# logv/sybil

Hardware: AMD Instinct MI355X
Metric: rows scanned/sec (1B-row x 32-int-col synthetic table, 3 ANDed int-range filters, group-by 2 cols, count/sum/avg/stddev of 2 cols) (higher is better)
Workload: dtype int64

## Files before the change

### sybil_amd/csrc/engine.cpp

```cpp
#include "engine.h"
#include "hll.h"
#include "re2lite.h"

#include <math.h>
#include <stdarg.h>
#include <stdio.h>
#include <stdlib.h>
#include <string.h>

#include <algorithm>
#include <mutex>
#include <unordered_map>
#include <string>
#include <vector>
#include <regex>

namespace sybl {

extern "C" char **environ;
const char *env(const char *name) {
    static std::unordered_map<std::string, std::string> snap;
    static bool live = false;
    static std::once_flag once;
    std::call_once(once, [] {
// ... 60 lines not shown
    if (e != hipSuccess) return e;
    return hipStreamCreateWithPriority(out, hipStreamNonBlocking, toward < 0 ? greatest : least);
}

static void free_query(Query *q) {
    if (!q) return;
    if (!q->table_gone) {
        query_finish_lazy_results(q);
        if (q->t) {
            auto &v = q->t->queries;
            v.erase(std::remove(v.begin(), v.end(), q), v.end());
        }
    }
    q->eff_weight.reset();
    q->fword.reset();
    if (q->d_plan) hipFree(q->d_plan);
    if (q->d_preplan) hipFree(q->d_preplan);
    if (q->d_prebits) hipFree(q->d_prebits);
    if (q->d_segs) hipFree(q->d_segs);
    if (q->d_wg_seg_begin) hipFree(q->d_wg_seg_begin);
    if (q->d_pieces) hipFree(q->d_pieces);
    if (q->d_piece_queue) hipFree(q->d_piece_queue);
    if (q->d_wg_cell_base) hipFree(q->d_wg_cell_base);
    if (q->d_recs) hipFree(q->d_recs);
    if (q->d_h32) hipFree(q->d_h32);
    if (q->d_cursor) hipFree(q->d_cursor);
    for (void *p : q->d_idmasks) hipFree(p);
    if (q->own_partials) {
        if (q->d_sum) hipFree(q->d_sum);
        if (q->d_max) hipFree(q->d_max);
// ... 645 lines not shown
```

### sybil_amd/csrc/engine.h

```cpp
#pragma once
#include <hip/hip_runtime.h>
#include <stdint.h>

#include <map>
#include <atomic>
#include <functional>
#include <memory>
#include <mutex>
#include <string>
#include <unordered_map>
#include <string.h>
#include <stdio.h>
#include <stdlib.h>
#include <algorithm>
#include <chrono>
#include <thread>
#include <vector>

#include "../../include/sybilgpu.h"
#include "plan.h"
#include "scan_fast.h"
#include "scan_packed.h"
#include "fword.h"

// ... 118 lines not shown
    std::vector<int64_t> h_set_off;
    std::vector<int32_t> h_set_vals;
    bool set_dirty = false;
    void *d_stage = nullptr;
    int64_t stage_cap = 0;
};

struct LoadedBlock {
    std::string name;
    int64_t mtime_ns = 0, size = 0;
    int64_t index = -1;
};

struct FilterWord {
    std::vector<int> cols;
    int n = 0;
    int32_t bits[kFwordMaxFields] = {}, shift[kFwordMaxFields] = {};
    int elem[kFwordMaxFields] = {};
    int64_t vbase[kFwordMaxFields] = {};
    void *d_data = nullptr;
    int64_t cap_rows = 0;
    int64_t rows = 0, version = -1, blocks = 0;
    uint64_t planned = 0;
    ~FilterWord() {
        if (d_data) (void)hipFree(d_data);
    }
};

struct Query;
struct Table {
// ... 12 lines not shown
    int64_t scratch_words = 0;
    int64_t version = 0;
    int64_t broken_blocks = 0;
    sybl_load_stats load_stats{};
    sybl_digest_stats digest_stats{};
    sybl_select_stats select_stats{};
    sybl_concat_stats concat_stats{};
    sybl_lookup_stats lookup_stats{};
    sybl_compute_stats compute_stats{};
    std::string src_dir;
    int src_rank = 0, src_nranks = 1;
    std::vector<LoadedBlock> loaded;
    std::vector<Query *> queries;
    std::vector<std::shared_ptr<FilterWord>> fwords;
    uint64_t fword_clock = 0;
    Column *find(const char *name) const;
};

int table_ensure_stats(Table *t);
int table_reserve(Table *t, Column *c, int64_t phys_rows);
int valid_reserve(Table *t, Column *c, int64_t phys_rows);
int64_t table_drop_dead_tail(Table *t, int64_t keep_blocks);
int table_upload_blocks(Table *t);
int table_reclaim_dead_rows(Table *t, bool force);
void column_free(Column *c);
int32_t dict_intern(Column *c, const std::string &s);
int column_upload_set(Table *t, Column *c);
int column_build_gdict(Table *t, Column *c);
int column_build_rank(Table *t, Column *c);
Column *column_build_narrow(Table *t, Column *c);
void column_drop_narrow(Column *c);
std::shared_ptr<FilterWord> table_build_fword(Table *t, const int *cols, int n);
int column_install_gdict(Table *t, Column *c);
int column_repack(Table *t, Column *c, int width, int64_t vbase);

struct BlockWriter {
    Table *t = nullptr;
    int64_t start = 0, nrows = 0, new_phys = 0;
    struct Staged {
        Column *c = nullptr;
        bool have_stats = false;
        int64_t mn = 0, mx = 0, pop = 0;
    };
    std::vector<Staged> staged;
    std::vector<Staged> direct;
    bool serial = false;
};
// ... 140 lines not shown
    ScanPlan dplan;
    ScanPlan *d_dplan = nullptr;
    uint8_t *d_hll = nullptr;
    uint64_t *d_hll_idhash = nullptr;
    char *d_hll_chars = nullptr;
    int64_t *d_hll_stroff = nullptr;
    int64_t hll_bytes = 0;
    bool distinct_pending = false;
    bool time_mode = false;
    int64_t time_bucket = 0;
    std::string order_by;
    bool order_asc = false;
    int limit = 0;
    std::shared_ptr<Column> eff_weight;
    std::shared_ptr<FilterWord> fword;
    int printed_level = 0;
    bool printed_only = false;
    bool top_only = false;
    bool top_merge = false;
    std::vector<GroupInfo> groups;
    std::vector<AggInfo> aggs;
    ScanPlan plan;
    ScanPlan *d_plan = nullptr;
    bool plan_dirty = true;
    int n_wg = 0;
    bool use_lds = false;
    size_t lds_bytes = 0;
    int64_t group_cells = 0;
    std::vector<Segment> segs;
    std::vector<int32_t> wg_seg_begin;
// ... 171 lines not shown
```

### sybil_amd/csrc/fword.h

```cpp
#pragma once
#ifdef __HIPCC__
#include <hip/hip_runtime.h>
#endif
#include <stdint.h>

#ifndef SYBL_HD
#ifdef __HIPCC__
#define SYBL_HD __host__ __device__ __forceinline__
#else
#define SYBL_HD inline
#endif
#endif

namespace sybl {

constexpr int kFwordMaxFields = 4;
constexpr int kFwordMinFields = 2;
constexpr int kFwordBits = 32;

SYBL_HD int fword_bits(uint32_t max_off) {
    int b = 1;
    while (b < 32 && (max_off >> b) != 0) b++;
    return b;
}
// ... 6 lines not shown
        total += bits[i];
    }
    return total;
}

SYBL_HD uint32_t fword_mask(int bits) { return (1u << bits) - 1u; }

SYBL_HD uint32_t fword_pack(const uint32_t *offsets, int n, const int32_t *shifts) {
    uint32_t w = 0;
    for (int i = 0; i < n; i++) w |= offsets[i] << shifts[i];
    return w;
}

SYBL_HD uint32_t fword_field(uint32_t word, int shift, int bits) { return (word >> shift) & fword_mask(bits); }

struct FwordPack {
    const void *col[kFwordMaxFields];
    int32_t wid[kFwordMaxFields];
    int32_t shift[kFwordMaxFields], bits[kFwordMaxFields];
    int32_t n;
};

}
```

### sybil_amd/csrc/planner.cpp

```cpp
#include <math.h>
#include <stdlib.h>
#include <string.h>

#include <algorithm>

#include "engine.h"
#include "hll.h"
#include "re2lite.h"

namespace sybl {

static inline int64_t round_up(int64_t x, int64_t m) { return (x + m - 1) / m * m; }


struct HostFilterFold {
    bool has_range = false;
    int64_t lo = INT64_MIN, hi = INT64_MAX;
    std::vector<int64_t> neq;
    bool has_mask = false;
    std::vector<uint8_t> mask;
    std::vector<std::pair<int32_t, int32_t>> setp;
};

static void setup_buckets(int64_t info_min, int64_t info_max, int64_t hist_bucket, int64_t *bucket_size,
// ... 1539 lines not shown
            if (cols[c] < 0) return;
            const Column *col = t->cols[(size_t)cols[c]].get();
            if (FP.fmask[c] || FP.nneq[c] || FP.npneq[c] || FP.fvalid[c] || FP.fwid[c] != col->elem || FP.fbase[c] != col->vbase) return;
        }
        std::shared_ptr<FilterWord> w = table_build_fword(t, cols, q->fast_nf);
        if (!w) return;
        for (int c = 0; c < q->fast_nf; c++) {
            const int i = (int)(std::find(w->cols.begin(), w->cols.end(), cols[c]) - w->cols.begin());
            FP.fshift[c] = w->shift[i];
            FP.fbits[c] = w->bits[i];
        }
        FP.fword = (const uint32_t *)w->d_data;
        q->fword = std::move(w);
    }

    void plan_narrow() {
        if (!(q->fast && q->fast_packed && !q->fast_packed_n && !q->hash_mode && !q->part_hist)) return;
        FastPlan &FP = q->fplan;
        plan_fword();
        for (int a = 0; a < q->fast_na; a++) {
            Column *c = t->cols[(size_t)q->aggs[(size_t)a].col].get();
            if (FP.awid[a] != 4 || (const void *)FP.acol[a] != c->d_data || FP.abase[a] != c->vbase) continue;
            if (Column *n = column_build_narrow(t, c)) {
                FP.acol[a] = (const int64_t *)n->d_data;
                FP.awid[a] = n->elem;
            }
        }
        if (env("SYBL_PLAN_TRACE")) {
            int bytes = q->time_mode ? FP.twid : 0;
            for (int c = 0; c < q->fast_nf; c++) bytes += FP.fword ? 0 : FP.fwid[c];
            for (int c = 0; c < q->fast_ng; c++) bytes += FP.gwid[c];
            std::string line = "narrow:";
            if (FP.fword) {
                bytes += 4;
                line += " f=word(";
                for (int c = 0; c < q->fast_nf; c++) line += (c ? "," : "") + std::to_string(FP.fbits[c]);
                line += ")";
            }
            for (int a = 0; a < q->fast_na; a++) {
                bytes += FP.awid[a];
                line += " a" + std::to_string(a) + "=" + std::to_string(FP.awid[a]);
            }
            fprintf(stderr, "%s bytes_per_row=%d\n", line.c_str(), bytes);
        }
    }

    int plan_pushdown() {
        q->pushdown = false;
        q->pd_static = q->printed_level == 2 && !env("SYBL_NO_PUSHDOWN") && !env("SYBL_NO_PUSHDOWN_RANKS") && q->limit > 0 && q->order_by == "$COUNT" &&
                       !q->order_asc && d->n_groups == 1 && d->n_filters == 0 && d->op == SYBL_AGG_HIST && d->n_aggs >= 1 && d->n_aggs <= 2 &&
                       d->n_distincts == 0 && ctx->comm && ctx->comm_nranks > 1;
        q->pd_agreed = -1;
        if (q->printed_level != 2 || env("SYBL_NO_PUSHDOWN")) return SYBL_OK;
        if (!q->part_hist || !q->part_packed || !q->part_more.empty() || q->part_nf != 0 || q->part_ng != 1) return SYBL_OK;
// ... 379 lines not shown
```

### sybil_amd/csrc/scan_fast.h

```cpp
#pragma once
#include <hip/hip_runtime.h>
#include <stdint.h>

#include "plan.h"
#include "pieces.h"
#include "outlog.h"
#include "wg_header.h"

namespace sybl {

constexpr int kFastMaxF = 4, kFastMaxG = 4, kFastMaxA = 4;
constexpr int kFastTemplatedG = 2, kFastTemplatedA = 2;

enum FastMode : int {
    kFastAvg = 0,
    kFastAvgMax = 1,
    kFastMoments = 2,
    kFastHist = 3,
    kFastModes = 4,
};

struct FastPlan {
    const int64_t *fcol[kFastMaxF];
    const int64_t *gcol[kFastMaxG];
// ... 44 lines not shown
    int32_t nul;
    int32_t lds_sum_fields;
    const int32_t *wg_cell_base;
    const uint32_t *xvalid;
    int64_t *out_log;
    int64_t out_cap;
    int64_t *sum_out, *max_out, *ws_sum, *ws_max;
    const Segment *segs;
    const int32_t *wg_seg_begin;
    unsigned long long *wg_clock;
    int32_t dyn, n_pieces, piece_cap;
    const Piece *pieces;
    uint32_t *piece_queue;
    const uint32_t *fword;
    int32_t fshift[kFastMaxF], fbits[kFastMaxF];
};

hipError_t launch_scan_fast(const FastPlan &P, int nf, int ng, int na, int mode, bool time, bool gen, int n_wg,
                            size_t lds_bytes, hipStream_t st);

inline bool fast_plan_has_narrow(const FastPlan &P, bool aggs) {
    bool any = P.twid == 3 || P.wwid == 3;
    for (int c = 0; c < kFastMaxF; c++) any = any || P.fwid[c] == 3;
    for (int c = 0; c < kFastMaxG; c++) any = any || P.gwid[c] == 3;
    for (int c = 0; aggs && c < kFastMaxA; c++) any = any || P.awid[c] == 3;
    return any;
}

constexpr uint32_t kLeanMoments = 1u, kLeanProved = 2u;
constexpr int lean_sum_fields(int na) { return na + (na + 1) / 2 + na; }
constexpr int lean_bits(unsigned __int128 x) {
    int b = 0;
    while (x) b++, x >>= 1;
    return b;
}
constexpr int lean_moments_fit(int na, const uint64_t *umax, const uint64_t *bmax, unsigned __int128 slot_rows) {
    const unsigned __int128 one = 1;
// ... 1103 lines not shown
```

### sybil_amd/csrc/scan_packed.h

```cpp
#pragma once
#include "narrow3.h"
#include "fword.h"
#include "scan_fast.h"

namespace sybl {

constexpr int kPackedRows = 4;
constexpr int kPackedTileRows = kWgThreads * kPackedRows;

hipError_t launch_scan_packed(const FastPlan &P, int nf, int ng, int na, int mode, bool time, int n_wg, size_t lds_bytes,
                              hipStream_t st);
hipError_t launch_emit_packed(const EmitPlan &E, int nf, int ng, int na, int n_wg, hipStream_t st);
hipError_t launch_count_packed_nf0(const EmitPlan &E, int ng, int n_wg, hipStream_t st);
hipError_t launch_count_packed_nf1(const EmitPlan &E, int ng, int n_wg, hipStream_t st);
hipError_t launch_count_packed_nf2(const EmitPlan &E, int ng, int n_wg, hipStream_t st);
hipError_t launch_count_packed_nf3(const EmitPlan &E, int ng, int n_wg, hipStream_t st);
hipError_t launch_count_packed_nf4(const EmitPlan &E, int ng, int n_wg, hipStream_t st);
hipError_t launch_emit_packed_nf0(const EmitPlan &E, int ng, int na, int n_wg, hipStream_t st);
hipError_t launch_emit_packed_nf1(const EmitPlan &E, int ng, int na, int n_wg, hipStream_t st);
hipError_t launch_emit_packed_nf2(const EmitPlan &E, int ng, int na, int n_wg, hipStream_t st);
hipError_t launch_emit_packed_nf3(const EmitPlan &E, int ng, int na, int n_wg, hipStream_t st);
hipError_t launch_emit_packed_nf4(const EmitPlan &E, int ng, int na, int n_wg, hipStream_t st);
hipError_t launch_scan_packed_nf0(const FastPlan &P, int ng, int na, int mode, bool time, int n_wg, size_t lds, hipStream_t st);
hipError_t launch_scan_packed_nf1(const FastPlan &P, int ng, int na, int mode, bool time, int n_wg, size_t lds, hipStream_t st);
// ... 421 lines not shown
            want_draw = false;
        }
    }
    __device__ __forceinline__ DynTile next() {
        if (left == 0 && !done) enter_piece();
        DynTile T;
        T.R = ((int64_t)__builtin_amdgcn_readfirstlane((int)(R >> 32)) << 32) | (uint32_t)__builtin_amdgcn_readfirstlane((int)(uint32_t)R);
        left = __builtin_amdgcn_readfirstlane(left);
        T.rows = left < (uint32_t)kPackedTileRows ? left : (uint32_t)kPackedTileRows;
        R = T.R + kPackedTileRows;
        left -= T.rows;
        return T;
    }
};

template <int NF, int NG, int NA, int MODE, bool TIME, bool G1, int LEANV, bool FW>
__device__ __forceinline__ void packed_scan_dyn(const FastPlan &P, int64_t *lds, const FastLds &L, const bool max32, uint32_t &matched,
                                                uint32_t &overflow) {
    static_assert(!FW || NF >= kFwordMinFields, "a filter word holds at least two columns");
    static_assert(kFwordMaxFields == kFastMaxF, "one field per filter column of a FastPlan");
    __shared__ uint32_t ring[4];
    const uint32_t tid = threadIdx.x;
    const uint32_t wave_row = __builtin_amdgcn_readfirstlane((tid & ~63u) * kPackedRows);
    const uint32_t lane_row = (tid & 63u) * kPackedRows;
    DynCursor cur(P, ring);
    PackedRaw<NF> rf;
    PackedRaw<NG> rg;
    PackedRaw<NA> ra;
    PackedRaw<1> rt;
    PackedTile<NF> f;
    PackedTile<NG> g;
    PackedTile<NA> a;
    PackedTile<1> t;
    auto issue = [&](const void *col, int width, const DynTile &T, bool wanted, pu32x4 &raw, bool one_dword) {
        const uint32_t rows = wanted && T.rows > wave_row
// ... 17 lines not shown
    auto decode_filters = [&]() {
        if constexpr (FW) {
            const uint32_t wd[kPackedRows] = {rf.v[0].x, rf.v[0].y, rf.v[0].z, rf.v[0].w};
#pragma unroll
            for (int c = 0; c < NF; c++) {
#pragma unroll
                for (int k = 0; k < kPackedRows; k++) f.u[c][k] = __builtin_amdgcn_ubfe(wd[k], (uint32_t)P.fshift[c], (uint32_t)P.fbits[c]);
            }
        } else {
#pragma unroll
            for (int c = 0; c < NF; c++) packed_decode(P.fwid[c], rf.v[c], f.u[c]);
        }
    };
    auto issue_rest = [&](const DynTile &T, bool wanted) {
        if (TIME) issue(P.tcol, P.twid, T, wanted, rt.v[0], false);
#pragma unroll
        for (int c = 0; c < NG; c++) issue(P.gcol[c], G1 ? 1 : P.gwid[c], T, wanted, rg.v[c], G1);
#pragma unroll
        for (int c = 0; c < NA; c++) issue(P.acol[c], P.awid[c], T, wanted, ra.v[c], false);
    };
    auto decode_rest = [&]() {
        if (TIME) packed_decode(P.twid, rt.v[0], t.u[0]);
#pragma unroll
        for (int c = 0; c < NG; c++) packed_decode(G1 ? 1 : P.gwid[c], rg.v[c], g.u[c]);
#pragma unroll
        for (int c = 0; c < NA; c++) packed_decode(P.awid[c], ra.v[c], a.u[c]);
    };
    auto lane_left = [&](const DynTile &T) -> uint32_t { return T.rows > tid * kPackedRows ? T.rows - tid * kPackedRows : 0u; };
    if (kPackedLate && NF > 0 && NG + NA + (TIME ? 1 : 0) > 0) {
        PackedTile<0> f0;
        auto filter_bits = [&](const DynTile &T) -> uint32_t {
            decode_filters();
            const uint32_t left = lane_left(T);
            uint32_t bits = 0;
#pragma unroll
            for (int k = 0; k < kPackedRows; k++) {
                bool pass = (uint32_t)k < left;
#pragma unroll
                for (int c = 0; c < NF; c++) pass = pass & (f.u[c][k] >= P.plo[c]) & (f.u[c][k] <= P.phi[c]);
                bits |= pass ? 1u << k : 0u;
            }
// ... 32 lines not shown
    cur.draw_ahead();
    while (T0.rows) {
        decode_filters();
        decode_rest();
        const DynTile T1 = cur.next();
        issue_filters(T1);
        issue_rest(T1, true);
        cur.draw_ahead();
        const uint32_t left = lane_left(T0);
        if (NF == 0) matched += left < (uint32_t)kPackedRows ? left : (uint32_t)kPackedRows;
        packed_plain_tile<NF, NG, NA, MODE, TIME, false, NF == 0, LEANV>(P, f, g, a, t, [&](int k) { return (uint32_t)k < left; }, lds, L, max32,
                                                                        matched, overflow);
        T0 = T1;
    }
}
template <int NF, int NG, int NA, int MODE, bool TIME, bool G1, bool NUL, int RING = 0, int LEANV = 0, bool DYN = false, bool FW = false>
__global__ __launch_bounds__(kWgThreads, SYBL_PACKED_WAVES_PER_EU) void k_scan_packed(const FastPlan P) {
    static_assert(LEANV == 0 || !NUL, "the NUL kernels mix row bodies: no proofs");
    static_assert(!DYN || (!NUL && RING == 0), "dynamic dealing is the plain kernels'");
    static_assert(!FW || (DYN && NF >= kFwordMinFields), "filter words are the dynamic loops', for two filter columns and more");
    static_assert(!(LEANV & kLeanMoments) || (MODE == kFastMoments && NA >= 1), "the lean layout is moments mode's");
    static_assert(!(LEANV & kLeanProved) || MODE == kFastMoments || MODE == kFastHist, "the proved bodies are the bucket modes'");
    extern __shared__ int64_t lds[];
    const uint32_t tid = threadIdx.x;
    constexpr bool kMax32 = MODE == kFastAvgMax && !NUL;
    constexpr bool lean_layout = (LEANV & kLeanMoments) != 0;
    const FastLds L = fast_begin<MODE>(P, lds, kMax32 && !P.ext_general, lean_layout);

    uint32_t matched = 0, overflow = 0;
    const uint64_t clock_in = P.wg_clock ? wall_clock64() : 0;
    if constexpr (DYN) packed_scan_dyn<NF, NG, NA, MODE, TIME, G1, LEANV, FW>(P, lds, L, kMax32 && !P.ext_general, matched, overflow);
    const int s0 = DYN ? 0 : P.wg_seg_begin[blockIdx.x], s1 = DYN ? 0 : P.wg_seg_begin[blockIdx.x + 1];
    for (int si = s0; si < s1; si++) {
        const Segment seg = P.segs[si];
        for (int64_t c0 = 0; c0 < seg.n; c0 += kPackedChunkRows) {
            const int64_t first = seg.start + c0;
            const uint32_t n = (uint32_t)(seg.n - c0 < kPackedChunkRows ? seg.n - c0 : kPackedChunkRows);
            PackedBases<NF, NG, NA> B;
#pragma unroll
            for (int c = 0; c < NF; c++) B.f[c] = (const uint8_t *)P.fcol[c] + first * P.fwid[c];
#pragma unroll
            for (int c = 0; c < NG; c++) B.g[c] = (const uint8_t *)P.gcol[c] + first * P.gwid[c];
#pragma unroll
            for (int c = 0; c < NA; c++) B.a[c] = (const uint8_t *)P.acol[c] + first * P.awid[c];
            B.t = TIME ? (const uint8_t *)P.tcol + first * P.twid : nullptr;
            B.first = first;
// ... 570 lines not shown
        }
    }
#undef SYBL_EMITL_CASE
    switch (ng * 3 + na) {
        SYBL_EMITP_CASE(0, 1)
        SYBL_EMITP_CASE(0, 2)
        SYBL_EMITP_CASE(1, 1)
        SYBL_EMITP_CASE(1, 2)
        SYBL_EMITP_CASE(2, 1)
        SYBL_EMITP_CASE(2, 2)
    default: return hipErrorInvalidValue;
    }
#undef SYBL_EMITP_CASE
}

template <int NF, int NG, int NA, int MODE, bool TIME, bool G1, bool FW, class LAUNCH>
static hipError_t packed_launch_dyn(const FastPlan &P, LAUNCH &&launch_lean) {
    if constexpr (NA >= 1 && MODE == kFastMoments) {
        switch (P.lean) {
        case 0: return launch_lean(k_scan_packed<NF, NG, NA, MODE, TIME, G1, false, 0, 0, true, FW>);
        case kLeanMoments: return launch_lean(k_scan_packed<NF, NG, NA, MODE, TIME, G1, false, 0, kLeanMoments, true, FW>);
        case kLeanProved: return launch_lean(k_scan_packed<NF, NG, NA, MODE, TIME, G1, false, 0, kLeanProved, true, FW>);
        case kLeanMoments | kLeanProved: return launch_lean(k_scan_packed<NF, NG, NA, MODE, TIME, G1, false, 0, kLeanMoments | kLeanProved, true, FW>);
        default: return hipErrorInvalidValue;
        }
    } else if constexpr (NA >= 1 && MODE == kFastHist) {
        if (P.lean == kLeanProved) return launch_lean(k_scan_packed<NF, NG, NA, MODE, TIME, G1, false, 0, kLeanProved, true, FW>);
        if (P.lean) return hipErrorInvalidValue;
        return launch_lean(k_scan_packed<NF, NG, NA, MODE, TIME, G1, false, 0, 0, true, FW>);
    } else {
        if (P.lean) return hipErrorInvalidValue;
        return launch_lean(k_scan_packed<NF, NG, NA, MODE, TIME, G1, false, 0, 0, true, FW>);
    }
}

template <int NF, int NG, int NA, int MODE, bool TIME, bool G1, bool NUL>
static hipError_t packed_launch_k1(const FastPlan &P, int n_wg, size_t lds_bytes, hipStream_t st) {
    constexpr bool kAb = !NUL && ((NF == 3 && NG == 2 && NA == 2 && MODE == kFastMoments && !TIME && G1) ||
                                  (NF == 0 && NG == 1 && NA == 2 && MODE == kFastAvgMax && !TIME && G1) ||
                                  (NF == 0 && NG == 1 && NA == 1 && MODE == kFastAvg && TIME && !G1));
    auto launch_lean = [&](auto kern) {
        hipError_t e2 = hipFuncSetAttribute((const void *)kern, hipFuncAttributeMaxDynamicSharedMemorySize, (int)lds_bytes);
        if (e2 != hipSuccess) return e2;
        hipLaunchKernelGGL(kern, dim3(n_wg), dim3(kWgThreads), lds_bytes, st, P);
        return hipGetLastError();
    };
    if (P.dyn) {
        if constexpr (!NUL) {
            if (!P.pieces || !P.piece_queue || P.n_pieces < 1 || P.piece_cap < 1) return hipErrorInvalidValue;
            if (P.fword) {
                if constexpr (NF >= kFwordMinFields) {
                    for (int c = 0; c < NF; c++)
                        if (P.fbits[c] < 1 || P.fshift[c] < 0 || P.fshift[c] + P.fbits[c] > kFwordBits) return hipErrorInvalidValue;
                    return packed_launch_dyn<NF, NG, NA, MODE, TIME, G1, true>(P, launch_lean);
                } else {
                    return hipErrorInvalidValue;
                }
            }
            return packed_launch_dyn<NF, NG, NA, MODE, TIME, G1, false>(P, launch_lean);
        } else {
            return hipErrorInvalidValue;
        }
    }
    if (P.fword) return hipErrorInvalidValue;
    if (P.lean) {
        if constexpr (!NUL && NA >= 1 && MODE == kFastMoments) {
            switch (P.lean) {
            case kLeanMoments: return launch_lean(k_scan_packed<NF, NG, NA, MODE, TIME, G1, NUL, 0, kLeanMoments>);
            case kLeanProved: return launch_lean(k_scan_packed<NF, NG, NA, MODE, TIME, G1, NUL, 0, kLeanProved>);
            case kLeanMoments | kLeanProved: return launch_lean(k_scan_packed<NF, NG, NA, MODE, TIME, G1, NUL, 0, kLeanMoments | kLeanProved>);
            default: return hipErrorInvalidValue;
            }
        } else if constexpr (!NUL && NA >= 1 && MODE == kFastHist) {
            if (P.lean != kLeanProved) return hipErrorInvalidValue;
            return launch_lean(k_scan_packed<NF, NG, NA, MODE, TIME, G1, NUL, 0, kLeanProved>);
        } else {
            return hipErrorInvalidValue;
        }
    }
// ... 66 lines not shown
```

### sybil_amd/csrc/table.cpp

```cpp
#include <string.h>

#include <algorithm>

#include "derived.h"

namespace sybl {

int host_to_device(Ctx *ctx, void *dst, const void *src, size_t bytes, const char *what) {
    if (bytes == 0) return SYBL_OK;
    constexpr size_t kPiece = (size_t)4 << 20;
    hipStream_t st = ctx->stream;
    if (!ctx->h2d_stage) {
        SYBL_HIP(hipHostMalloc((void **)&ctx->h2d_stage, kPiece, hipHostMallocDefault));
        ctx->h2d_stage_bytes = kPiece;
    }
    for (size_t at = 0; at < bytes; at += kPiece) {
        const size_t n = std::min(kPiece, bytes - at);
        memcpy(ctx->h2d_stage, (const char *)src + at, n);
        SYBL_HIP(hipMemcpyAsync((char *)dst + at, ctx->h2d_stage, n, hipMemcpyHostToDevice, st));
        SYBL_HIP(hipStreamSynchronize(st));
    }
    if (!env("SYBL_VERIFY_COPIES")) return SYBL_OK;
    if (bytes % 4) return fail(SYBL_E_INVAL, "host_to_device(%s): %zu bytes are not whole words", what, bytes);
    if (!ctx->d_copy_digest) SYBL_HIP(hipMalloc((void **)&ctx->d_copy_digest, 8));
// ... 774 lines not shown
    if (trace)
        fprintf(stderr, "narrow twin: col=%s rows=%lld converted=%lld bytes=%lld\n", c->name.c_str(), (long long)t->phys_rows,
                (long long)(t->phys_rows - from), (long long)(r->cap_rows * kNarrowWidth));
    c->narrow_rows = t->phys_rows;
    c->narrow_version = t->version;
    c->narrow_blocks = (int64_t)t->blocks.size();
    return r;
}

static std::string fword_list(const Table *t, const FilterWord &w, bool names) {
    std::string s;
    for (int i = 0; i < w.n; i++) s += (i ? "," : "") + (names ? t->cols[(size_t)w.cols[(size_t)i]]->name : std::to_string(w.bits[i]));
    return s;
}

std::shared_ptr<FilterWord> table_build_fword(Table *t, const int *cols_in, int n) {
    if (n < kFwordMinFields || n > kFwordMaxFields) return nullptr;
    std::vector<int> cols(cols_in, cols_in + n);
    std::sort(cols.begin(), cols.end());
    if (std::adjacent_find(cols.begin(), cols.end()) != cols.end() || cols.front() < 0 || cols.back() >= (int)t->cols.size()) return nullptr;
    int64_t min_rows = (int64_t)1 << 25, max_words = 2;
    if (const char *e = env("SYBL_FWORD_MIN_ROWS")) min_rows = std::max<int64_t>(atoll(e), 1);
    if (const char *e = env("SYBL_FWORD_MAX")) max_words = std::max<int64_t>(atoll(e), 1);
    const bool trace = env("SYBL_PLAN_TRACE") != nullptr;
    auto held = [&]() { return std::find_if(t->fwords.begin(), t->fwords.end(), [&](const std::shared_ptr<FilterWord> &w) { return w->cols == cols; }); };
    auto drop = [&](bool say) {
        auto it = held();
        if (it == t->fwords.end()) return;
        if (say && trace) fprintf(stderr, "filter word: cols=%s freed\n", fword_list(t, **it, true).c_str());
        t->fwords.erase(it);
    };
    auto it = held();
    const bool current = it != t->fwords.end() && (*it)->version == t->version;
    if (env("SYBL_NO_FWORD") || t->phys_rows < min_rows) {
        if (it != t->fwords.end() && !current) drop(false);
        return nullptr;
    }
    if (current) {
        (*it)->planned = ++t->fword_clock;
        return *it;
    }
    if (table_ensure_stats(t) != SYBL_OK) return nullptr;
    uint32_t max_off[kFwordMaxFields];
    int32_t bits[kFwordMaxFields], shift[kFwordMaxFields];
    int widths = 0;
    bool eligible = true;
    for (int i = 0; i < n && eligible; i++) {
        const Column *c = t->cols[(size_t)cols[(size_t)i]].get();
        eligible = c->type == SYBL_INT_VAL && (c->elem == 1 || c->elem == 2 || c->elem == 4) && c->d_data && c->n_pop > 0 && c->exact_min >= c->vbase &&
                   !c->has_missing && (unsigned __int128)((__int128)c->exact_max - (__int128)c->vbase) <= (unsigned __int128)UINT32_MAX;
        if (!eligible) break;
        max_off[i] = (uint32_t)((uint64_t)c->exact_max - (uint64_t)c->vbase);
        widths += c->elem;
    }
    eligible = eligible && fword_layout(max_off, n, bits, shift) <= kFwordBits && widths >= 5;
    if (!eligible) {
        drop(true);
        return nullptr;
    }
    std::shared_ptr<FilterWord> w = it != t->fwords.end() ? *it : nullptr;
    int64_t from = 0;
    if (w) {
        bool same = true, fits = true;
        for (int i = 0; i < n; i++) {
            const Column *c = t->cols[(size_t)cols[(size_t)i]].get();
            same = same && w->elem[i] == c->elem && w->vbase[i] == c->vbase;
            fits = fits && bits[i] <= w->bits[i];
        }
        if (same && fits && w->rows <= t->phys_rows && (int64_t)t->blocks.size() >= w->blocks && t->version - w->version == (int64_t)t->blocks.size() - w->blocks)
            from = w->rows & ~(int64_t)3;
        if (from == 0) {
            drop(same && !fits);
            w.reset();
            if (same && !fits) return nullptr;
        }
    }
    hipStream_t st = t->ctx->stream;
    auto give_up = [&]() -> std::shared_ptr<FilterWord> {
        (void)hipGetLastError();
        drop(false);
        return nullptr;
    };
    if (load_sync_all(t->ctx) != SYBL_OK) return give_up();
    const int64_t need = t->phys_rows + kTileRows;
    if (!w || need > w->cap_rows) {
        auto nw = std::make_shared<FilterWord>();
        nw->cols = cols;
        nw->n = n;
        for (int i = 0; i < n; i++) {
            const Column *c = t->cols[(size_t)cols[(size_t)i]].get();
            nw->bits[i] = w ? w->bits[i] : bits[i];
            nw->shift[i] = w ? w->shift[i] : shift[i];
            nw->elem[i] = c->elem;
            nw->vbase[i] = c->vbase;
        }
        if (!w)
            while ((int64_t)t->fwords.size() >= max_words) {
                auto lru = std::min_element(t->fwords.begin(), t->fwords.end(),
                                            [](const std::shared_ptr<FilterWord> &a, const std::shared_ptr<FilterWord> &b) { return a->planned < b->planned; });
                if (trace) fprintf(stderr, "filter word: cols=%s freed\n", fword_list(t, **lru, true).c_str());
                t->fwords.erase(lru);
            }
        const int64_t cap = w ? std::max(need, w->cap_rows + w->cap_rows / 2) : need;
        if (hipMalloc(&nw->d_data, (size_t)cap * 4) != hipSuccess) {
            nw->d_data = nullptr;
            return give_up();
        }
        nw->cap_rows = cap;
        if (w && from > 0) {
            if (hipMemcpyAsync(nw->d_data, w->d_data, (size_t)from * 4, hipMemcpyDeviceToDevice, st) != hipSuccess || hipStreamSynchronize(st) != hipSuccess) return give_up();
        }
        if (w) drop(false);
        t->fwords.push_back(nw);
        w = nw;
    }
    FwordPack S;
    memset(&S, 0, sizeof(S));
    S.n = n;
    for (int i = 0; i < n; i++) {
        const Column *c = t->cols[(size_t)cols[(size_t)i]].get();
        S.col[i] = c->d_data;
        S.wid[i] = c->elem;
        S.shift[i] = w->shift[i];
        S.bits[i] = w->bits[i];
    }
    hipError_t e = launch_pack_fword(S, w->d_data, from, t->phys_rows - from, st);
    if (e == hipSuccess) e = hipStreamSynchronize(st);
    if (e != hipSuccess) return give_up();
    if (trace)
        fprintf(stderr, "filter word: cols=%s bits=%s rows=%lld converted=%lld bytes=%lld\n", fword_list(t, *w, true).c_str(), fword_list(t, *w, false).c_str(),
                (long long)t->phys_rows, (long long)(t->phys_rows - from), (long long)(w->cap_rows * 4));
    w->rows = t->phys_rows;
    w->version = t->version;
    w->blocks = (int64_t)t->blocks.size();
    w->planned = ++t->fword_clock;
    return w;
}

int column_upload_set(Table *t, Column *c) {
    if (c->type != SYBL_SET_VAL || !c->set_dirty) return SYBL_OK;
    if (c->h_set_off.empty()) c->h_set_off.push_back(0);
    std::vector<int64_t> off = c->h_set_off;
    while ((int64_t)off.size() < t->phys_rows + kTileRows + 2) off.push_back(off.back());
    if (c->d_set_off) SYBL_HIP(hipFree(c->d_set_off));
    if (c->d_set_vals) SYBL_HIP(hipFree(c->d_set_vals));
// ... 170 lines not shown

int64_t sybl_table_rows(const sybl_table *t) { SYBL_API_GUARD(t); return t ? t->logical_rows : 0; }
int64_t sybl_table_blocks(const sybl_table *t) { SYBL_API_GUARD(t); return t ? (int64_t)t->blocks.size() : 0; }

int64_t sybl_table_hbm_bytes(const sybl_table *t) {
    SYBL_API_GUARD(t);
    if (!t) return 0;
    int64_t b = 0;
    for (auto &c : t->cols) {
        b += c->cap_rows * c->elem + c->valid_cap_words * 4 + c->set_vals_cap * 4;
        if (c->rank_col) b += c->rank_col->cap_rows * c->rank_col->elem;
        if (c->carried_weight) b += c->carried_weight->cap_rows * c->carried_weight->elem;
        if (c->narrow) b += c->narrow->cap_rows * c->narrow->elem;
    }
    for (auto &w : t->fwords) b += w->cap_rows * 4;
    return b;
}

int sybl_table_column_info(const sybl_table *tc, const char *name, int *type, int64_t *exact_min, int64_t *exact_max,
                           int64_t *info_min, int64_t *info_max, int *has_missing) {
    SYBL_API_GUARD(tc);
    sybl_table *t = const_cast<sybl_table *>(tc);
    if (!t) return fail(SYBL_E_INVAL, "table is NULL");
    Column *c = t->find(name);
    if (!c) return fail(SYBL_E_INVAL, "unknown column '%s'", name ? name : "(null)");
    SYBL_HIP(hipSetDevice(t->ctx->device));
    int rc = table_ensure_stats(t);
    if (rc) return rc;
    if (type) *type = c->type;
    if (exact_min) *exact_min = c->exact_min;
// ... 188 lines not shown
```

Measured before the change: 497.6 billion.

## Pack group keys and first aggregate into a cached 32-bit key word

```diff
diff --git a/sybil_amd/csrc/engine.cpp b/sybil_amd/csrc/engine.cpp
--- a/sybil_amd/csrc/engine.cpp
+++ b/sybil_amd/csrc/engine.cpp
@@ -98,6 +98,7 @@
     }
     q->eff_weight.reset();
     q->fword.reset();
+    q->kword.reset();
     if (q->d_plan) hipFree(q->d_plan);
     if (q->d_preplan) hipFree(q->d_preplan);
     if (q->d_prebits) hipFree(q->d_prebits);
diff --git a/sybil_amd/csrc/engine.h b/sybil_amd/csrc/engine.h
--- a/sybil_amd/csrc/engine.h
+++ b/sybil_amd/csrc/engine.h
@@ -156,6 +156,7 @@
 
 struct FilterWord {
     std::vector<int> cols;
+    int agg = -1;
     int n = 0;
     int32_t bits[kFwordMaxFields] = {}, shift[kFwordMaxFields] = {};
     int elem[kFwordMaxFields] = {};
@@ -198,6 +199,7 @@
     std::vector<Query *> queries;
     std::vector<std::shared_ptr<FilterWord>> fwords;
     uint64_t fword_clock = 0;
+    std::vector<std::shared_ptr<FilterWord>> kwords;
     Column *find(const char *name) const;
 };
 
@@ -215,6 +217,7 @@
 Column *column_build_narrow(Table *t, Column *c);
 void column_drop_narrow(Column *c);
 std::shared_ptr<FilterWord> table_build_fword(Table *t, const int *cols, int n);
+std::shared_ptr<FilterWord> table_build_kword(Table *t, const int *keys, int n_keys, int agg);
 int column_install_gdict(Table *t, Column *c);
 int column_repack(Table *t, Column *c, int width, int64_t vbase);
 
@@ -385,6 +388,7 @@
     int limit = 0;
     std::shared_ptr<Column> eff_weight;
     std::shared_ptr<FilterWord> fword;
+    std::shared_ptr<FilterWord> kword;
     int printed_level = 0;
     bool printed_only = false;
     bool top_only = false;
diff --git a/sybil_amd/csrc/fword.h b/sybil_amd/csrc/fword.h
--- a/sybil_amd/csrc/fword.h
+++ b/sybil_amd/csrc/fword.h
@@ -44,6 +44,8 @@
 
 SYBL_HD uint32_t fword_field(uint32_t word, int shift, int bits) { return (word >> shift) & fword_mask(bits); }
 
+SYBL_HD int word_bytes_today(int elem, uint32_t max_off, bool is_agg) { return is_agg && elem == 4 && max_off < (1u << 24) ? 3 : elem; }
+
 struct FwordPack {
     const void *col[kFwordMaxFields];
     int32_t wid[kFwordMaxFields];
diff --git a/sybil_amd/csrc/planner.cpp b/sybil_amd/csrc/planner.cpp
--- a/sybil_amd/csrc/planner.cpp
+++ b/sybil_amd/csrc/planner.cpp
@@ -1577,11 +1577,45 @@
         q->fword = std::move(w);
     }
 
+    void plan_kword() {
+        FastPlan &FP = q->fplan;
+        FP.kword = nullptr;
+        q->kword.reset();
+        if (!kPackedLate || !q->dyn || FP.nul || P.windowed || q->time_mode || q->fast_nf < 1 || q->fast_ng < 1 || q->fast_na < 1) return;
+        if (q->fast_ng + 1 > kFwordMaxFields || q->fast_ng > kFastTemplatedG || q->fast_na > kFastTemplatedA) return;
+        if ((q->fast_nf >= kFwordMinFields) != (FP.fword != nullptr)) return;
+        if (FP.wcol || FP.f_out[0] >= 0 || FP.f_cnt[0] >= 0 || FP.f_pop[0] >= 0 || FP.avalid[0]) return;
+        auto stored = [&](const void *p, int wid, int64_t base) -> int {
+            for (size_t i = 0; i < t->cols.size(); i++)
+                if (t->cols[i]->d_data && t->cols[i]->d_data == p) return wid == t->cols[i]->elem && base == t->cols[i]->vbase ? (int)i : -1;
+            return -1;
+        };
+        int keys[kFastMaxG];
+        for (int c = 0; c < q->fast_ng; c++) {
+            keys[c] = FP.gvalid[c] ? -1 : stored(FP.gcol[c], FP.gwid[c], FP.gbase[c]);
+            if (keys[c] < 0) return;
+        }
+        const int agg = stored(FP.acol[0], FP.awid[0], FP.abase[0]);
+        if (agg < 0) return;
+        std::shared_ptr<FilterWord> w = table_build_kword(t, keys, q->fast_ng, agg);
+        if (!w) return;
+        auto field = [&](int col) { return (int)(std::find(w->cols.begin(), w->cols.end(), col) - w->cols.begin()); };
+        for (int c = 0; c < q->fast_ng; c++) {
+            FP.gshift[c] = w->shift[field(keys[c])];
+            FP.gbits[c] = w->bits[field(keys[c])];
+        }
+        FP.kashift = w->shift[field(agg)];
+        FP.kabits = w->bits[field(agg)];
+        FP.kword = (const uint32_t *)w->d_data;
+        q->kword = std::move(w);
+    }
+
     void plan_narrow() {
         if (!(q->fast && q->fast_packed && !q->fast_packed_n && !q->hash_mode && !q->part_hist)) return;
         FastPlan &FP = q->fplan;
         plan_fword();
-        for (int a = 0; a < q->fast_na; a++) {
+        plan_kword();
+        for (int a = FP.kword ? 1 : 0; a < q->fast_na; a++) {
             Column *c = t->cols[(size_t)q->aggs[(size_t)a].col].get();
             if (FP.awid[a] != 4 || (const void *)FP.acol[a] != c->d_data || FP.abase[a] != c->vbase) continue;
             if (Column *n = column_build_narrow(t, c)) {
@@ -1592,7 +1626,7 @@
         if (env("SYBL_PLAN_TRACE")) {
             int bytes = q->time_mode ? FP.twid : 0;
             for (int c = 0; c < q->fast_nf; c++) bytes += FP.fword ? 0 : FP.fwid[c];
-            for (int c = 0; c < q->fast_ng; c++) bytes += FP.gwid[c];
+            for (int c = 0; c < q->fast_ng; c++) bytes += FP.kword ? 0 : FP.gwid[c];
             std::string line = "narrow:";
             if (FP.fword) {
                 bytes += 4;
@@ -1600,7 +1634,13 @@
                 for (int c = 0; c < q->fast_nf; c++) line += (c ? "," : "") + std::to_string(FP.fbits[c]);
                 line += ")";
             }
-            for (int a = 0; a < q->fast_na; a++) {
+            if (FP.kword) {
+                bytes += 4;
+                line += " k=word(";
+                for (int c = 0; c < q->fast_ng; c++) line += std::to_string(FP.gbits[c]) + ",";
+                line += std::to_string(FP.kabits) + ")";
+            }
+            for (int a = FP.kword ? 1 : 0; a < q->fast_na; a++) {
                 bytes += FP.awid[a];
                 line += " a" + std::to_string(a) + "=" + std::to_string(FP.awid[a]);
             }
diff --git a/sybil_amd/csrc/scan_fast.h b/sybil_amd/csrc/scan_fast.h
--- a/sybil_amd/csrc/scan_fast.h
+++ b/sybil_amd/csrc/scan_fast.h
@@ -82,13 +82,15 @@
     uint32_t *piece_queue;
     const uint32_t *fword;
     int32_t fshift[kFastMaxF], fbits[kFastMaxF];
+    const uint32_t *kword;
+    int32_t gshift[kFastMaxG], gbits[kFastMaxG], kashift, kabits;
 };
 
 hipError_t launch_scan_fast(const FastPlan &P, int nf, int ng, int na, int mode, bool time, bool gen, int n_wg,
                             size_t lds_bytes, hipStream_t st);
 
 inline bool fast_plan_has_narrow(const FastPlan &P, bool aggs) {
-    bool any = P.twid == 3 || P.wwid == 3;
+    bool any = P.twid == 3 || P.wwid == 3 || (aggs && P.kword != nullptr);
     for (int c = 0; c < kFastMaxF; c++) any = any || P.fwid[c] == 3;
     for (int c = 0; c < kFastMaxG; c++) any = any || P.gwid[c] == 3;
     for (int c = 0; aggs && c < kFastMaxA; c++) any = any || P.awid[c] == 3;
diff --git a/sybil_amd/csrc/scan_packed.h b/sybil_amd/csrc/scan_packed.h
--- a/sybil_amd/csrc/scan_packed.h
+++ b/sybil_amd/csrc/scan_packed.h
@@ -459,11 +459,14 @@
     }
 };
 
-template <int NF, int NG, int NA, int MODE, bool TIME, bool G1, int LEANV, bool FW>
+template <int NF, int NG, int NA, int MODE, bool TIME, bool G1, int LEANV, bool FW, bool KW>
 __device__ __forceinline__ void packed_scan_dyn(const FastPlan &P, int64_t *lds, const FastLds &L, const bool max32, uint32_t &matched,
                                                 uint32_t &overflow) {
     static_assert(!FW || NF >= kFwordMinFields, "a filter word holds at least two columns");
     static_assert(kFwordMaxFields == kFastMaxF, "one field per filter column of a FastPlan");
+    static_assert(!KW || (!TIME && !G1 && NF >= 1 && NG >= 1 && NA >= 1), "a key word holds the keys and aggregation 0 of the late loop");
+    static_assert(!KW || kPackedLate, "a key word is read by the late loop");
+    static_assert(!KW || NG + 1 <= kFwordMaxFields, "one field per key column and one for aggregation 0");
     __shared__ uint32_t ring[4];
     const uint32_t tid = threadIdx.x;
     const uint32_t wave_row = __builtin_amdgcn_readfirstlane((tid & ~63u) * kPackedRows);
@@ -511,17 +514,32 @@
     };
     auto issue_rest = [&](const DynTile &T, bool wanted) {
         if (TIME) issue(P.tcol, P.twid, T, wanted, rt.v[0], false);
-#pragma unroll
-        for (int c = 0; c < NG; c++) issue(P.gcol[c], G1 ? 1 : P.gwid[c], T, wanted, rg.v[c], G1);
-#pragma unroll
-        for (int c = 0; c < NA; c++) issue(P.acol[c], P.awid[c], T, wanted, ra.v[c], false);
+        if constexpr (KW) {
+            issue(P.kword, 4, T, wanted, ra.v[0], false);
+        } else {
+#pragma unroll
+            for (int c = 0; c < NG; c++) issue(P.gcol[c], G1 ? 1 : P.gwid[c], T, wanted, rg.v[c], G1);
+        }
+#pragma unroll
+        for (int c = KW ? 1 : 0; c < NA; c++) issue(P.acol[c], P.awid[c], T, wanted, ra.v[c], false);
     };
     auto decode_rest = [&]() {
         if (TIME) packed_decode(P.twid, rt.v[0], t.u[0]);
-#pragma unroll
-        for (int c = 0; c < NG; c++) packed_decode(G1 ? 1 : P.gwid[c], rg.v[c], g.u[c]);
-#pragma unroll
-        for (int c = 0; c < NA; c++) packed_decode(P.awid[c], ra.v[c], a.u[c]);
+        if constexpr (KW) {
+            const uint32_t wd[kPackedRows] = {ra.v[0].x, ra.v[0].y, ra.v[0].z, ra.v[0].w};
+#pragma unroll
+            for (int c = 0; c < NG; c++) {
+#pragma unroll
+                for (int k = 0; k < kPackedRows; k++) g.u[c][k] = __builtin_amdgcn_ubfe(wd[k], (uint32_t)P.gshift[c], (uint32_t)P.gbits[c]);
+            }
+#pragma unroll
+            for (int k = 0; k < kPackedRows; k++) a.u[0][k] = __builtin_amdgcn_ubfe(wd[k], (uint32_t)P.kashift, (uint32_t)P.kabits);
+        } else {
+#pragma unroll
+            for (int c = 0; c < NG; c++) packed_decode(G1 ? 1 : P.gwid[c], rg.v[c], g.u[c]);
+        }
+#pragma unroll
+        for (int c = KW ? 1 : 0; c < NA; c++) packed_decode(P.awid[c], ra.v[c], a.u[c]);
     };
     auto lane_left = [&](const DynTile &T) -> uint32_t { return T.rows > tid * kPackedRows ? T.rows - tid * kPackedRows : 0u; };
     if (kPackedLate && NF > 0 && NG + NA + (TIME ? 1 : 0) > 0) {
@@ -584,11 +602,14 @@
         T0 = T1;
     }
 }
-template <int NF, int NG, int NA, int MODE, bool TIME, bool G1, bool NUL, int RING = 0, int LEANV = 0, bool DYN = false, bool FW = false>
+template <int NF, int NG, int NA, int MODE, bool TIME, bool G1, bool NUL, int RING = 0, int LEANV = 0, bool DYN = false, bool FW = false,
+          bool KW = false>
 __global__ __launch_bounds__(kWgThreads, SYBL_PACKED_WAVES_PER_EU) void k_scan_packed(const FastPlan P) {
     static_assert(LEANV == 0 || !NUL, "the NUL kernels mix row bodies: no proofs");
     static_assert(!DYN || (!NUL && RING == 0), "dynamic dealing is the plain kernels'");
     static_assert(!FW || (DYN && NF >= kFwordMinFields), "filter words are the dynamic loops', for two filter columns and more");
+    static_assert(!KW || (DYN && !TIME && !G1 && NG >= 1 && NA >= 1 && FW == (NF >= kFwordMinFields) && NF >= 1),
+                  "key words are the dynamic late loop's: keys and an aggregation, one filter column or a filter word");
     static_assert(!(LEANV & kLeanMoments) || (MODE == kFastMoments && NA >= 1), "the lean layout is moments mode's");
     static_assert(!(LEANV & kLeanProved) || MODE == kFastMoments || MODE == kFastHist, "the proved bodies are the bucket modes'");
     extern __shared__ int64_t lds[];
@@ -599,7 +620,7 @@
 
     uint32_t matched = 0, overflow = 0;
     const uint64_t clock_in = P.wg_clock ? wall_clock64() : 0;
-    if constexpr (DYN) packed_scan_dyn<NF, NG, NA, MODE, TIME, G1, LEANV, FW>(P, lds, L, kMax32 && !P.ext_general, matched, overflow);
+    if constexpr (DYN) packed_scan_dyn<NF, NG, NA, MODE, TIME, G1, LEANV, FW, KW>(P, lds, L, kMax32 && !P.ext_general, matched, overflow);
     const int s0 = DYN ? 0 : P.wg_seg_begin[blockIdx.x], s1 = DYN ? 0 : P.wg_seg_begin[blockIdx.x + 1];
     for (int si = s0; si < s1; si++) {
         const Segment seg = P.segs[si];
@@ -1200,23 +1221,23 @@
 #undef SYBL_EMITP_CASE
 }
 
-template <int NF, int NG, int NA, int MODE, bool TIME, bool G1, bool FW, class LAUNCH>
+template <int NF, int NG, int NA, int MODE, bool TIME, bool G1, bool FW, bool KW, class LAUNCH>
 static hipError_t packed_launch_dyn(const FastPlan &P, LAUNCH &&launch_lean) {
     if constexpr (NA >= 1 && MODE == kFastMoments) {
         switch (P.lean) {
-        case 0: return launch_lean(k_scan_packed<NF, NG, NA, MODE, TIME, G1, false, 0, 0, true, FW>);
-        case kLeanMoments: return launch_lean(k_scan_packed<NF, NG, NA, MODE, TIME, G1, false, 0, kLeanMoments, true, FW>);
-        case kLeanProved: return launch_lean(k_scan_packed<NF, NG, NA, MODE, TIME, G1, false, 0, kLeanProved, true, FW>);
-        case kLeanMoments | kLeanProved: return launch_lean(k_scan_packed<NF, NG, NA, MODE, TIME, G1, false, 0, kLeanMoments | kLeanProved, true, FW>);
+        case 0: return launch_lean(k_scan_packed<NF, NG, NA, MODE, TIME, G1, false, 0, 0, true, FW, KW>);
+        case kLeanMoments: return launch_lean(k_scan_packed<NF, NG, NA, MODE, TIME, G1, false, 0, kLeanMoments, true, FW, KW>);
+        case kLeanProved: return launch_lean(k_scan_packed<NF, NG, NA, MODE, TIME, G1, false, 0, kLeanProved, true, FW, KW>);
+        case kLeanMoments | kLeanProved: return launch_lean(k_scan_packed<NF, NG, NA, MODE, TIME, G1, false, 0, kLeanMoments | kLeanProved, true, FW, KW>);
         default: return hipErrorInvalidValue;
         }
     } else if constexpr (NA >= 1 && MODE == kFastHist) {
-        if (P.lean == kLeanProved) return launch_lean(k_scan_packed<NF, NG, NA, MODE, TIME, G1, false, 0, kLeanProved, true, FW>);
+        if (P.lean == kLeanProved) return launch_lean(k_scan_packed<NF, NG, NA, MODE, TIME, G1, false, 0, kLeanProved, true, FW, KW>);
         if (P.lean) return hipErrorInvalidValue;
-        return launch_lean(k_scan_packed<NF, NG, NA, MODE, TIME, G1, false, 0, 0, true, FW>);
+        return launch_lean(k_scan_packed<NF, NG, NA, MODE, TIME, G1, false, 0, 0, true, FW, KW>);
     } else {
         if (P.lean) return hipErrorInvalidValue;
-        return launch_lean(k_scan_packed<NF, NG, NA, MODE, TIME, G1, false, 0, 0, true, FW>);
+        return launch_lean(k_scan_packed<NF, NG, NA, MODE, TIME, G1, false, 0, 0, true, FW, KW>);
     }
 }
 
@@ -1238,17 +1259,30 @@
                 if constexpr (NF >= kFwordMinFields) {
                     for (int c = 0; c < NF; c++)
                         if (P.fbits[c] < 1 || P.fshift[c] < 0 || P.fshift[c] + P.fbits[c] > kFwordBits) return hipErrorInvalidValue;
-                    return packed_launch_dyn<NF, NG, NA, MODE, TIME, G1, true>(P, launch_lean);
                 } else {
                     return hipErrorInvalidValue;
                 }
             }
-            return packed_launch_dyn<NF, NG, NA, MODE, TIME, G1, false>(P, launch_lean);
+            if (P.kword) {
+                if constexpr (kPackedLate && !TIME && NF >= 1 && NG >= 1 && NA >= 1) {
+                    if ((P.fword != nullptr) != (NF >= kFwordMinFields)) return hipErrorInvalidValue;
+                    for (int c = 0; c < NG; c++)
+                        if (P.gbits[c] < 1 || P.gshift[c] < 0 || P.gshift[c] + P.gbits[c] > kFwordBits) return hipErrorInvalidValue;
+                    if (P.kabits < 1 || P.kashift < 0 || P.kashift + P.kabits > kFwordBits) return hipErrorInvalidValue;
+                    return packed_launch_dyn<NF, NG, NA, MODE, TIME, false, (NF >= kFwordMinFields), true>(P, launch_lean);
+                } else {
+                    return hipErrorInvalidValue;
+                }
+            }
+            if constexpr (NF >= kFwordMinFields) {
+                if (P.fword) return packed_launch_dyn<NF, NG, NA, MODE, TIME, G1, true, false>(P, launch_lean);
+            }
+            return packed_launch_dyn<NF, NG, NA, MODE, TIME, G1, false, false>(P, launch_lean);
         } else {
             return hipErrorInvalidValue;
         }
     }
-    if (P.fword) return hipErrorInvalidValue;
+    if (P.fword || P.kword) return hipErrorInvalidValue;
     if (P.lean) {
         if constexpr (!NUL && NA >= 1 && MODE == kFastMoments) {
             switch (P.lean) {
diff --git a/sybil_amd/csrc/table.cpp b/sybil_amd/csrc/table.cpp
--- a/sybil_amd/csrc/table.cpp
+++ b/sybil_amd/csrc/table.cpp
@@ -812,26 +812,46 @@
     return s;
 }
 
-std::shared_ptr<FilterWord> table_build_fword(Table *t, const int *cols_in, int n) {
+struct WordKind {
+    std::vector<std::shared_ptr<FilterWord>> Table::*list;
+    const char *label, *env_min_rows, *env_max, *env_off;
+};
+static const WordKind kFilterWords = {&Table::fwords, "filter word", "SYBL_FWORD_MIN_ROWS", "SYBL_FWORD_MAX", "SYBL_NO_FWORD"};
+static const WordKind kKeyWords = {&Table::kwords, "key word", "SYBL_KWORD_MIN_ROWS", "SYBL_KWORD_MAX", "SYBL_NO_KWORD"};
+
+static std::shared_ptr<FilterWord> table_build_word(Table *t, const int *cols_in, int n, int agg, const WordKind &K);
+
+std::shared_ptr<FilterWord> table_build_fword(Table *t, const int *cols, int n) { return table_build_word(t, cols, n, -1, kFilterWords); }
+
+std::shared_ptr<FilterWord> table_build_kword(Table *t, const int *keys, int n_keys, int agg) {
+    if (n_keys < 1 || n_keys + 1 > kFwordMaxFields || agg < 0) return nullptr;
+    int cols[kFwordMaxFields];
+    for (int i = 0; i < n_keys; i++) cols[i] = keys[i];
+    cols[n_keys] = agg;
+    return table_build_word(t, cols, n_keys + 1, agg, kKeyWords);
+}
+
+static std::shared_ptr<FilterWord> table_build_word(Table *t, const int *cols_in, int n, int agg, const WordKind &K) {
+    std::vector<std::shared_ptr<FilterWord>> &words = t->*(K.list);
     if (n < kFwordMinFields || n > kFwordMaxFields) return nullptr;
     std::vector<int> cols(cols_in, cols_in + n);
     std::sort(cols.begin(), cols.end());
     if (std::adjacent_find(cols.begin(), cols.end()) != cols.end() || cols.front() < 0 || cols.back() >= (int)t->cols.size()) return nullptr;
     int64_t min_rows = (int64_t)1 << 25, max_words = 2;
-    if (const char *e = env("SYBL_FWORD_MIN_ROWS")) min_rows = std::max<int64_t>(atoll(e), 1);
-    if (const char *e = env("SYBL_FWORD_MAX")) max_words = std::max<int64_t>(atoll(e), 1);
+    if (const char *e = env(K.env_min_rows)) min_rows = std::max<int64_t>(atoll(e), 1);
+    if (const char *e = env(K.env_max)) max_words = std::max<int64_t>(atoll(e), 1);
     const bool trace = env("SYBL_PLAN_TRACE") != nullptr;
-    auto held = [&]() { return std::find_if(t->fwords.begin(), t->fwords.end(), [&](const std::shared_ptr<FilterWord> &w) { return w->cols == cols; }); };
+    auto held = [&]() { return std::find_if(words.begin(), words.end(), [&](const std::shared_ptr<FilterWord> &w) { return w->cols == cols && w->agg == agg; }); };
     auto drop = [&](bool say) {
         auto it = held();
-        if (it == t->fwords.end()) return;
-        if (say && trace) fprintf(stderr, "filter word: cols=%s freed\n", fword_list(t, **it, true).c_str());
-        t->fwords.erase(it);
+        if (it == words.end()) return;
+        if (say && trace) fprintf(stderr, "%s: cols=%s freed\n", K.label, fword_list(t, **it, true).c_str());
+        words.erase(it);
     };
     auto it = held();
-    const bool current = it != t->fwords.end() && (*it)->version == t->version;
-    if (env("SYBL_NO_FWORD") || t->phys_rows < min_rows) {
-        if (it != t->fwords.end() && !current) drop(false);
+    const bool current = it != words.end() && (*it)->version == t->version;
+    if (env(K.env_off) || t->phys_rows < min_rows) {
+        if (it != words.end() && !current) drop(false);
         return nullptr;
     }
     if (current) {
@@ -849,14 +869,14 @@
                    !c->has_missing && (unsigned __int128)((__int128)c->exact_max - (__int128)c->vbase) <= (unsigned __int128)UINT32_MAX;
         if (!eligible) break;
         max_off[i] = (uint32_t)((uint64_t)c->exact_max - (uint64_t)c->vbase);
-        widths += c->elem;
+        widths += word_bytes_today(c->elem, max_off[i], cols[(size_t)i] == agg);
     }
     eligible = eligible && fword_layout(max_off, n, bits, shift) <= kFwordBits && widths >= 5;
     if (!eligible) {
         drop(true);
         return nullptr;
     }
-    std::shared_ptr<FilterWord> w = it != t->fwords.end() ? *it : nullptr;
+    std::shared_ptr<FilterWord> w = it != words.end() ? *it : nullptr;
     int64_t from = 0;
     if (w) {
         bool same = true, fits = true;
@@ -884,6 +904,7 @@
     if (!w || need > w->cap_rows) {
         auto nw = std::make_shared<FilterWord>();
         nw->cols = cols;
+        nw->agg = agg;
         nw->n = n;
         for (int i = 0; i < n; i++) {
             const Column *c = t->cols[(size_t)cols[(size_t)i]].get();
@@ -893,11 +914,11 @@
             nw->vbase[i] = c->vbase;
         }
         if (!w)
-            while ((int64_t)t->fwords.size() >= max_words) {
-                auto lru = std::min_element(t->fwords.begin(), t->fwords.end(),
+            while ((int64_t)words.size() >= max_words) {
+                auto lru = std::min_element(words.begin(), words.end(),
                                             [](const std::shared_ptr<FilterWord> &a, const std::shared_ptr<FilterWord> &b) { return a->planned < b->planned; });
-                if (trace) fprintf(stderr, "filter word: cols=%s freed\n", fword_list(t, **lru, true).c_str());
-                t->fwords.erase(lru);
+                if (trace) fprintf(stderr, "%s: cols=%s freed\n", K.label, fword_list(t, **lru, true).c_str());
+                words.erase(lru);
             }
         const int64_t cap = w ? std::max(need, w->cap_rows + w->cap_rows / 2) : need;
         if (hipMalloc(&nw->d_data, (size_t)cap * 4) != hipSuccess) {
@@ -909,7 +930,7 @@
             if (hipMemcpyAsync(nw->d_data, w->d_data, (size_t)from * 4, hipMemcpyDeviceToDevice, st) != hipSuccess || hipStreamSynchronize(st) != hipSuccess) return give_up();
         }
         if (w) drop(false);
-        t->fwords.push_back(nw);
+        words.push_back(nw);
         w = nw;
     }
     FwordPack S;
@@ -926,7 +947,7 @@
     if (e == hipSuccess) e = hipStreamSynchronize(st);
     if (e != hipSuccess) return give_up();
     if (trace)
-        fprintf(stderr, "filter word: cols=%s bits=%s rows=%lld converted=%lld bytes=%lld\n", fword_list(t, *w, true).c_str(), fword_list(t, *w, false).c_str(),
+        fprintf(stderr, "%s: cols=%s bits=%s rows=%lld converted=%lld bytes=%lld\n", K.label, fword_list(t, *w, true).c_str(), fword_list(t, *w, false).c_str(),
                 (long long)t->phys_rows, (long long)(t->phys_rows - from), (long long)(w->cap_rows * 4));
     w->rows = t->phys_rows;
     w->version = t->version;
@@ -1127,6 +1148,7 @@
         if (c->narrow) b += c->narrow->cap_rows * c->narrow->elem;
     }
     for (auto &w : t->fwords) b += w->cap_rows * 4;
+    for (auto &w : t->kwords) b += w->cap_rows * 4;
     return b;
 }
 
```

Result: faster. 511.7 billion (median of 6 runs) (+2.9%).
